# ChASE-library/ChASE

Measured on AMD Instinct MI355X. Metric: chebyshev_filter_hemm_gflops, higher is better.
Workload: dtype complex f64

## Files before the change

### chase_amd/capi.py

```python
import ctypes as C
import os
import numpy as np

_HERE = os.path.dirname(os.path.abspath(__file__))
LIB_PATH = os.environ.get("CHASE_HIP_LIB") or os.path.join(_HERE, "lib", "libchase_hip.so")


class ChaseHipError(RuntimeError):
    def __init__(self, code, where, text=""):
        super().__init__(f"{where} failed with status {code}: {text}")
        self.code = code


def _load():
    if not os.path.exists(LIB_PATH):
        raise ImportError(
            f"{LIB_PATH} not found: build it with `make` (or `python -c 'import __graft_entry__ as g; g.build()'`). "
            "chase_amd has no CPU fallback.")
    try:
        import torch
    except Exception:
        pass
    return C.CDLL(LIB_PATH, mode=C.RTLD_GLOBAL)

# ... 166 lines not shown
        return DeviceArray(self, host.shape, dt).upload(host)

    def timer_start(self):
        check(lib.chase_hip_timer_start(self.h), "timer_start")

    def timer_stop(self):
        ms = C.c_float()
        check(lib.chase_hip_timer_stop(self.h, C.byref(ms)), "timer_stop")
        return ms.value

    def gemm(self, opA, m, n, k, alpha, A, lda, B, ldb, beta, Cm, ldc, cplx):
        op = opA.encode()[0:1]
        if cplx:
            check(lib.chase_hip_gemm_z(self.h, op, m, n, k, _z2(alpha), A, lda, B, ldb, _z2(beta), Cm, ldc), "gemm_z")
        else:
            check(lib.chase_hip_gemm_d(self.h, op, m, n, k, float(alpha), A, lda, B, ldb, float(beta), Cm, ldc),
                  "gemm_d")

    def gemm32(self, opA, m, n, k, alpha, A, lda, B, ldb, beta, Cm, ldc, cplx, split=False):
        op = opA.encode()[0:1]
        if cplx:
            f = lib.chase_hip_gemm_c_bf16x3 if split else lib.chase_hip_gemm_c
            check(f(self.h, op, m, n, k, _c2(alpha), A, lda, B, ldb, _c2(beta), Cm, ldc), "gemm_c")
        else:
            f = lib.chase_hip_gemm_s_bf16x3 if split else lib.chase_hip_gemm_s
            check(f(self.h, op, m, n, k, float(alpha), A, lda, B, ldb, float(beta), Cm, ldc), "gemm_s")

    def gemm32w(self, opA, m, n, k, alpha, A, lda, B, ldb, beta, Cm, ldc, cplx, split=False):
        op = opA.encode()[0:1]
        if cplx:
            f = lib.chase_hip_gemm_cz_bf16x3 if split else lib.chase_hip_gemm_cz
            check(f(self.h, op, m, n, k, _z2(alpha), A, lda, B, ldb, _z2(beta), Cm, ldc), "gemm_cz")
        else:
            f = lib.chase_hip_gemm_sd_bf16x3 if split else lib.chase_hip_gemm_sd
            check(f(self.h, op, m, n, k, float(alpha), A, lda, B, ldb, float(beta), Cm, ldc), "gemm_sd")

    def bf16x3_pack_bytes(self, m, k, cplx):
        b = c_size_t()
        check(lib.chase_hip_bf16x3_pack_bytes(int(cplx), m, k, C.byref(b)), "bf16x3_pack_bytes")
        return b.value

    def bf16x3_pack(self, m, k, A, lda, packed, cplx, src_f64=False):
        check(lib.chase_hip_bf16x3_pack(self.h, int(cplx), int(src_f64), m, k, A, lda, packed), "bf16x3_pack")

    def bf16x3_pack_diag(self, n, H64, ldh, packed, cplx):
        check(lib.chase_hip_bf16x3_pack_diag(self.h, int(cplx), n, H64, ldh, packed), "bf16x3_pack_diag")

    def gemm32p(self, m, n, k, alpha, packedA, B, ldb, beta, Cm, ldc, cplx):
        if cplx:
            check(lib.chase_hip_gemm_c_bf16x3p(self.h, m, n, k, _c2(alpha), packedA, B, ldb, _c2(beta), Cm, ldc), "gemm_c_bf16x3p")
        else:
            check(lib.chase_hip_gemm_s_bf16x3p(self.h, m, n, k, float(alpha), packedA, B, ldb, float(beta), Cm, ldc),
                  "gemm_s_bf16x3p")

    def set_gemm_min_rounds(self, rounds):
        check(lib.chase_hip_ctx_set_gemm_min_rounds(self.h, int(rounds)), "ctx_set_gemm_min_rounds")

    def gemm_sp_counters(self, reset=False):
        w, s, p = C.c_ulonglong(), C.c_ulonglong(), C.c_ulonglong()
        check(lib.chase_hip_ctx_gemm_sp_counters(self.h, C.byref(w), C.byref(s), C.byref(p), int(reset)), "ctx_gemm_sp_counters")
        return w.value, s.value, p.value

    def diag_list_d2s(self, H, ldh, Hs, ldhs, rows, cols, cnt, cplx):
        check(lib.chase_hip_diag_list_d2s(self.h, int(cplx), H, ldh, Hs, ldhs, rows, cols, cnt), "diag_list_d2s")

    def convert_d2s(self, m, n, src, ld_src, dst, ld_dst, cplx):
        check(lib.chase_hip_convert_d2s(self.h, int(cplx), m, n, src, ld_src, dst, ld_dst), "convert_d2s")

    def convert_s2d(self, m, n, src, ld_src, dst, ld_dst, cplx):
        check(lib.chase_hip_convert_s2d(self.h, int(cplx), m, n, src, ld_src, dst, ld_dst), "convert_s2d")

    def diag_d2s(self, n, H, ldh, Hs, ldhs, cplx):
        check(lib.chase_hip_diag_d2s(self.h, int(cplx), n, H, ldh, Hs, ldhs), "diag_d2s")

    def to_single(self, dA):
        cplx = dA.dtype == np.complex128
        out = self.empty(dA.shape, np.complex64 if cplx else np.float32)
        self.convert_d2s(dA.shape[0], dA.shape[1], dA.ptr, dA.ld, out.ptr, out.ld, cplx)
        return out

    def to_double(self, dA):
        cplx = dA.dtype == np.complex64
        out = self.empty(dA.shape, np.complex128 if cplx else np.float64)
        self.convert_s2d(dA.shape[0], dA.shape[1], dA.ptr, dA.ld, out.ptr, out.ld, cplx)
        return out

    def hash64(self, ptr, m, n, ld, cplx):
        h = C.c_ulonglong()
        check(lib.chase_hip_hash64(self.h, int(cplx), m, n, ptr, ld, C.byref(h)), "hash64")
        return h.value

    def gen_clement(self, N, cplx, scale=1.0, perturb=0.0, seed=42):
        dH = self.empty((N, N), np.complex128 if cplx else np.float64)
        check(lib.chase_hip_gen_clement(self.h, int(cplx), dH.ptr, N, N, N, N, N, 1, 0, 0, N, 1, 0, 0, float(scale),
                                        float(perturb), seed), "gen_clement")
        return dH

    def load_matrix(self, path, N, cplx):
        dH = self.empty((N, N), np.complex128 if cplx else np.float64)
        check(lib.chase_hip_load_matrix_shard(self.h, str(path).encode(), int(cplx), N, N, N, N, 1, 0, N, 1, 0, dH.ptr, N),
              "load_matrix_shard")
        return dH

    def save_matrix(self, path, dA):
        cplx = dA.dtype == np.complex128
        check(lib.chase_hip_save_matrix(self.h, str(path).encode(), int(cplx), dA.shape[0],
# ... 154 lines not shown


def tape_get(solver):
    p, n = P(c_double)(), c_size_t()
    check(lib.chase_hip_solver_tape_data(solver.h, C.byref(p), C.byref(n)), "tape_data")
    return np.ctypeslib.as_array(p, shape=(n.value,)).copy() if n.value else np.zeros(0)


def tape_load(solver, tape):
    t = np.ascontiguousarray(tape, dtype=np.float64)
    check(lib.chase_hip_solver_tape_load(solver.h, t.ctypes.data, t.size), "tape_load")


def gemm_counters(ctx, phase, reset=False):
    a, b, n = c_double(), c_double(), C.c_ulonglong()
    check(lib.chase_hip_ctx_gemm_counters(ctx.h, phase, C.byref(a), C.byref(b), C.byref(n), int(reset)), "gemm_counters")
    return a.value, b.value, n.value


class GemmLaunch(C.Structure):
    _fields_ = [(f, c_int) for f in ("row0", "col0", "k0", "m", "n", "k", "beta_one", "bn_cols", "narrow", "m3", "ragged",
                                     "glds_ok", "gm", "gn")] + \
               [("full_tiles", c_long), ("tail_tiles", c_long)] + \
               [(f, c_int) for f in ("tail_sk", "tail_kchunk", "group_rows", "forced_split")] + \
               [("slab_bytes", c_size_t), ("plane_bytes", c_size_t)]

    def as_dict(self):
        return {k: getattr(self, k) for k, _ in self._fields_}


_sig("chase_hip_gemm_plan", c_int, c_int, c_char, c_int, c_int, c_int, c_long, c_long, c_int, c_int, c_int, c_int,
     P(GemmLaunch), c_int)


def gemm_plan(cplx, op, m, n, k, lda=None, ldb=None, aligned=True, phase=0, num_cu=256, min_rounds=0):
    lda = (m if op == "N" else k) if lda is None else lda
    ldb = k if ldb is None else ldb
    args = (int(cplx), op.encode(), m, n, k, max(lda, 1), max(ldb, 1), int(aligned), phase, num_cu, min_rounds)
    cnt = lib.chase_hip_gemm_plan(*args, None, 0)
    if cnt < 0:
        check(cnt, "gemm_plan")
    out = (GemmLaunch * max(cnt, 1))()
    assert lib.chase_hip_gemm_plan(*args, out, cnt) == cnt
    return [out[i].as_dict() for i in range(cnt)]


class GemmSpLaunch(C.Structure):
    _fields_ = [(n, c_int) for n in ("bn", "gm", "gn", "sk", "kchunk", "min_piece_k")] + [("slab_bytes", c_size_t)]

    def as_dict(self):
        return {k: getattr(self, k) for k, _ in self._fields_}


_sig("chase_hip_gemm_sp_plan", c_int, c_int, c_int, c_char, c_int, c_int, c_int, c_int, c_int, P(GemmSpLaunch))
_sig("chase_hip_gemm_sp_workspace_bytes", c_size_t, c_int, c_int, c_char, c_int, c_int, c_int, c_int, c_int)
_sig("chase_hip_ctx_gemm_sp_counters", c_int, c_void_p, P(C.c_ulonglong), P(C.c_ulonglong), P(C.c_ulonglong), c_int)


def gemm_sp_plan(cplx, op, m, n, k, split=False, num_cu=256, min_rounds=0):
    out = GemmSpLaunch()
    check(lib.chase_hip_gemm_sp_plan(int(split), int(cplx), op.encode(), m, n, k, num_cu, min_rounds, C.byref(out)), "gemm_sp_plan")
    return out.as_dict()


def gemm_sp_workspace_bytes(cplx, op, m, n, k, split=False, num_cu=256, min_rounds=0):
    return lib.chase_hip_gemm_sp_workspace_bytes(int(split), int(cplx), op.encode(), m, n, k, num_cu, min_rounds)


class Solver:

    def __init__(self, ctx, H, nev, nex, V=None, h_on_device_ptr=None, N=None, cplx=None):
        self.ctx = ctx
        if h_on_device_ptr is None:
            assert H.flags.f_contiguous and H.ndim == 2 and H.shape[0] == H.shape[1]
            self.cplx = bool(np.iscomplexobj(H))
            self.N = H.shape[0]
            self.H = H
            hptr, on_dev = H.ctypes.data, 0
        else:
            self.cplx, self.N, self.H = bool(cplx), int(N), None
            hptr, on_dev = h_on_device_ptr, 1
        self.nev, self.nex = nev, nex
        dt = np.complex128 if self.cplx else np.float64
        self.V = np.zeros((self.N, nev + nex), dtype=dt, order="F") if V is None else V
        assert self.V.flags.f_contiguous and self.V.dtype == dt
        self.ritzv = np.zeros(nev + nex, dtype=np.float64)
        h = c_void_p()
        check(lib.chase_hip_solver_create(C.byref(h), ctx.h, int(self.cplx), self.N, nev, nex, hptr, self.N,
                                          self.V.ctypes.data, self.N, self.ritzv.ctypes.data, on_dev),
              "solver_create")
        self.h = h

    def close(self):
        if self.h:
            lib.chase_hip_solver_destroy(self.h)
            self.h = None

    def set(self, **kw):
        for k, v in kw.items():
            check(lib.chase_hip_solver_set(self.h, k.encode(), float(v)), f"solver_set({k})")

    def get(self, key):
        v = c_double()
        check(lib.chase_hip_solver_get(self.h, key.encode(), C.byref(v)), f"solver_get({key})")
        return v.value

# ... 125 lines not shown
```

### chase_amd/csrc/capi_core.hip

```cpp
#include <hip/hip_runtime.h>
#include <cstdlib>
#include <cstdio>
#include <cstring>
#include <string>
#include "../../include/chase_hip.h"
#include "ctx.h"
#include "kernels.h"
#include "gemm_sp_frame.h"

namespace chase_hip {
thread_local std::string g_last_error;
int set_error(int code, const char* what)
{
    g_last_error = what ? what : "";
    return code;
}
int hip_fail(hipError_t e, const char* where)
{
    char buf[512];
    snprintf(buf, sizeof buf, "%s: %s", where, hipGetErrorString(e));
    g_last_error = buf;
    return -(int)e;
}
}
// ... 262 lines not shown
}

int chase_hip_gemm_c_bf16x3(chase_hip_ctx* c, char opA, int m, int n, int k, const float alpha[2], const void* A, long lda,
                            const void* B, long ldb, const float beta[2], void* C, long ldc)
{
    if (!c) return set_error(CHASE_HIP_EINVAL, "ctx == NULL");
    if (!alpha || !beta) return set_error(CHASE_HIP_EINVAL, "gemm_c: NULL alpha/beta");
    return gemm32(c, true, opA, m, n, k, alpha, (const float*)A, lda, (const float*)B, ldb, beta, (float*)C, ldc, true);
}

int chase_hip_bf16x3_pack_bytes(int cplx, int m, int k, size_t* bytes)
{
    if (!bytes) return set_error(CHASE_HIP_EINVAL, "bf16x3_pack_bytes: bytes == NULL");
    if (m < 0 || k < 0) return set_error(CHASE_HIP_EINVAL, "bf16x3_pack_bytes: negative dimension");
    *bytes = bf16x3_pack_bytes(cplx != 0, m, k);
    return 0;
}

int chase_hip_bf16x3_pack(chase_hip_ctx* c, int cplx, int src_f64, int m, int k, const void* A, long lda, void* packed)
{
    if (!c) return set_error(CHASE_HIP_EINVAL, "bf16x3_pack: NULL ctx");
    (void)hipSetDevice(c->device);
    if (c->oplog_on) c->oplog_add("bf16x3_pack", m, k, 0, 0);
    if (m < 0 || k < 0 || lda < m) return set_error(CHASE_HIP_EINVAL, "bf16x3_pack: bad shape");
    if (m == 0 || k == 0) return 0;
    if (!A || !packed) return set_error(CHASE_HIP_EINVAL, "bf16x3_pack: NULL matrix");
    if (((uintptr_t)packed & 15) != 0) return set_error(CHASE_HIP_EINVAL, "bf16x3_pack: packed must be 16-byte aligned");
    int e = bf16x3_pack(c->stream, cplx != 0, src_f64 != 0, m, k, A, lda, packed);
    if (e) return hip_fail((hipError_t)e, "bf16x3_pack launch");
    return 0;
}

int chase_hip_bf16x3_pack_diag(chase_hip_ctx* c, int cplx, int n, const void* H64, long ldh, void* packed)
{
    if (!c) return set_error(CHASE_HIP_EINVAL, "bf16x3_pack_diag: NULL ctx");
    (void)hipSetDevice(c->device);
    if (c->oplog_on) c->oplog_add("bf16x3_pack_diag", n, 0, 0, 0);
    if (n < 0 || ldh < n) return set_error(CHASE_HIP_EINVAL, "bf16x3_pack_diag: bad shape");
    if (n == 0) return 0;
    if (!H64 || !packed) return set_error(CHASE_HIP_EINVAL, "bf16x3_pack_diag: NULL argument");
    int e = bf16x3_pack_diag(c->stream, cplx != 0, n, (const double*)H64, ldh, packed);
    if (e) return hip_fail((hipError_t)e, "bf16x3_pack_diag launch");
    return 0;
}

static int gemm32p(chase_hip_ctx* c, bool cplx, int m, int n, int k, const float* alpha, const void* packedA, const float* B, long ldb,
                   const float* beta, float* C, long ldc)
{
    (void)hipSetDevice(c->device);
    int rc = check_gemm('N', m, n, k, packedA, m, B, ldb, C, ldc);
    if (rc || m == 0 || n == 0) return rc;
    if (k > 0 && ((uintptr_t)packedA & 15) != 0) return set_error(CHASE_HIP_EINVAL, "gemm_bf16x3p: packedA must be 16-byte aligned");
    if (c->oplog_on) c->oplog_add(cplx ? "gemm_c3pN" : "gemm_s3pN", m, n, k, c->phase * 100);
    int e = gemm_bf16x3p(c->stream, cplx, m, n, k, alpha, packedA, B, ldb, beta, C, ldc, c->num_cu, c->phase == 1 ? 1 : 0);
    if (e) return hip_fail((hipError_t)e, "gemm_bf16x3p launch");
    return 0;
}

int chase_hip_gemm_s_bf16x3p(chase_hip_ctx* c, int m, int n, int k, float alpha, const void* packedA, const float* B, long ldb,
                             float beta, float* C, long ldc)
{
    if (!c) return set_error(CHASE_HIP_EINVAL, "ctx == NULL");
    return gemm32p(c, false, m, n, k, &alpha, packedA, B, ldb, &beta, C, ldc);
}

int chase_hip_gemm_c_bf16x3p(chase_hip_ctx* c, int m, int n, int k, const float alpha[2], const void* packedA, const void* B, long ldb,
                             const float beta[2], void* C, long ldc)
{
    if (!c) return set_error(CHASE_HIP_EINVAL, "ctx == NULL");
    if (!alpha || !beta) return set_error(CHASE_HIP_EINVAL, "gemm_c_bf16x3p: NULL alpha/beta");
    return gemm32p(c, true, m, n, k, alpha, packedA, (const float*)B, ldb, beta, (float*)C, ldc);
}

static int gemm32w(chase_hip_ctx* c, bool cplx, char opA, int m, int n, int k, const double* alpha, const float* A, long lda,
                   const float* B, long ldb, const double* beta, double* C, long ldc, bool split = false)
{
    (void)hipSetDevice(c->device);
    const bool opn = opA == 'N' || opA == 'n';
    const bool opc = opA == 'C' || opA == 'c' || (!cplx && (opA == 'T' || opA == 't'));
    if (!opn && !opc)
        return set_error(CHASE_HIP_EINVAL, cplx ? "gemm_cz: opA must be 'N' or 'C'" : "gemm_sd: opA must be 'N', 'C' or 'T'");
    int rc = check_gemm(opA, m, n, k, A, lda, B, ldb, C, ldc);
    if (rc || m == 0 || n == 0) return rc;
    if (c->oplog_on) {
        const char* name = split ? (cplx ? (opn ? "gemm_cz3N" : "gemm_cz3C") : (opn ? "gemm_sd3N" : "gemm_sd3C"))
                                 : (cplx ? (opn ? "gemm_czN" : "gemm_czC") : (opn ? "gemm_sdN" : "gemm_sdC"));
        c->oplog_add(name, m, n, k, c->phase * 100);
    }
    if (c->gemm_min_rounds > 0) {
        const size_t need = chase_hip_gemm_sp_workspace_bytes(split, cplx, opA, m, n, k, c->num_cu, c->gemm_min_rounds);
        if (need && (rc = c->ensure_ws((need + ((size_t)32 << 20) - 1) & ~(((size_t)32 << 20) - 1)))) return rc;
    }
    int pieces = 1;
    int e = (split ? gemm_bf16x3w : gemm_f32w)(c->stream, cplx, opA, m, n, k, alpha, A, lda, B, ldb, beta, C, ldc, c->num_cu,
                                               c->phase == 1 ? 1 : 0, (double*)c->ws, c->ws_bytes, c->gemm_min_rounds, &pieces);
    if (e == GEMM_F32_EOP) return set_error(CHASE_HIP_EINVAL, "gemm_sd / gemm_cz: bad opA");
    if (e == GEMM_F64_EWORKSPACE)
        return set_error(CHASE_HIP_EINVAL, "gemm_sd / gemm_cz: split-K workspace smaller than gemm_sp_workspace_bytes for this shape");
    if (e) return hip_fail((hipError_t)e, split ? "gemm_bf16x3w launch" : "gemm_f32w launch");
    ++c->sp_wide_calls;
    if (pieces > 1) { ++c->sp_split_calls; c->sp_pieces += (unsigned long long)pieces; }
    return 0;
}

int chase_hip_gemm_sd(chase_hip_ctx* c, char opA, int m, int n, int k, double alpha, const float* A, long lda, const float* B,
                      long ldb, double beta, double* C, long ldc)
{
    if (!c) return set_error(CHASE_HIP_EINVAL, "ctx == NULL");
// ... 146 lines not shown
```

### chase_amd/csrc/ctx.h

```cpp
#pragma once
#include <hip/hip_runtime.h>
#include <stddef.h>
#include <string>
#include <vector>

struct chase_hip_ctx {
    int device = 0;
    int num_cu = 0;
    int clock_khz = 0;
    size_t hbm_bytes = 0;
    char name[128] = {0};
    hipStream_t stream = nullptr;
    bool own_stream = false;
    hipEvent_t ev0 = nullptr, ev1 = nullptr;
    int phase = 0;
    double flops_model[4] = {0, 0, 0, 0}, flops_exec[4] = {0, 0, 0, 0};
    unsigned long long gemm_calls[4] = {0, 0, 0, 0};
    int gemm_min_rounds = 0;
    unsigned long long sp_wide_calls = 0, sp_split_calls = 0, sp_pieces = 0;
    void* ws = nullptr;
    size_t ws_bytes = 0;
    enum { BUF_TINV = 0, BUF_PANEL, BUF_SCAL, BUF_LAMBDA, BUF_RR, BUF_EIG, BUF_STEDC, BUF_APPLYQ, NBUF };
    void* bufs[NBUF] = {};
    size_t buf_bytes[NBUF] = {};
    void* hstage = nullptr;
    size_t hstage_bytes = 0;

    bool oplog_on = false;
    int oplog_mute = 0;
    std::vector<std::string> oplog;
    std::string oplog_text;
    void oplog_add(const char* name, long a, long b, long c, long d);

    int ensure_ws(size_t bytes);
    int ensure_buf(int idx, size_t bytes);
    int ensure_hstage(size_t bytes);
    int gemm(bool cplx, char opA, int m, int n, int k, const double* alpha, const double* A, long lda, const double* B,
             long ldb, const double* beta, double* C, long ldc);
};

namespace chase_hip {
int set_error(int code, const char* what);
int hip_fail(hipError_t e, const char* where);
}
```

### chase_amd/csrc/gemm_mfma_bf16x3p.hip

```cpp
#include "gemm_sp_frame.h"

namespace chase_hip {
namespace {

using namespace sp_frame;

typedef __bf16 bf16x8 __attribute__((ext_vector_type(8)));
typedef unsigned u32x4 __attribute__((ext_vector_type(4)));

constexpr int BK = 16;
constexpr int PA = 2 * BM;

__host__ __device__ __forceinline__ int piece(int row, int h) { return 2 * row + (h ^ (((row >> 2) ^ (row >> 3)) & 1)); }

__device__ __forceinline__ void split1(float v, __bf16& a1, __bf16& a2, __bf16& a3)
{
    a1 = (__bf16)v;
    const float r1 = v - (float)a1;
    a2 = (__bf16)r1;
    const float r2 = r1 - (float)a2;
    a3 = (__bf16)r2;
}

__device__ __forceinline__ void split3(const float* x, int st, u32x4& p1, u32x4& p2, u32x4& p3)
{
    bf16x8 a1, a2, a3;
    #pragma unroll
    for (int e = 0; e < 8; ++e) {
        __bf16 s1, s2, s3;
        split1(x[st * e], s1, s2, s3);
        a1[e] = s1; a2[e] = s2; a3[e] = s3;
    }
    p1 = __builtin_bit_cast(u32x4, a1); p2 = __builtin_bit_cast(u32x4, a2); p3 = __builtin_bit_cast(u32x4, a3);
}


template <bool CPLX, class S>
__global__ __launch_bounds__(256) void bf16x3_pack_kernel(int m, int k, const S* __restrict__ A, long lda, u32x4* __restrict__ out)
{
    constexpr int E = CPLX ? 2 : 1;
    const int tid = threadIdx.x, r = tid % BM, h = tid / BM;
    const long t = blockIdx.x, T = gridDim.x, p = blockIdx.y;
    const long row = p * BM + r, kg = t * BK + 8 * h;
    float x[8 * E];
    #pragma unroll
    for (int e = 0; e < 8; ++e) {
        #pragma unroll
        for (int c = 0; c < E; ++c) x[E * e + c] = 0.f;
        if (row < m && kg + e < k) {
            const S* q = A + E * (row + (kg + e) * lda);
            #pragma unroll
            for (int c = 0; c < E; ++c) x[E * e + c] = (float)q[c];
        }
    }
    u32x4* d = out + (p * T + t) * (3 * E * PA) + piece(r, h);
    #pragma unroll
    for (int c = 0; c < E; ++c) {
        u32x4 p1, p2, p3;
        split3(x + c, E, p1, p2, p3);
        d[(3 * c) * PA] = p1; d[(3 * c + 1) * PA] = p2; d[(3 * c + 2) * PA] = p3;
    }
}

template <bool CPLX>
__global__ __launch_bounds__(256) void bf16x3_pack_diag_kernel(int n, const double* __restrict__ H, long ldh, unsigned short* __restrict__ out)
{
    constexpr int E = CPLX ? 2 : 1;
    const long i = (long)blockIdx.x * 256 + threadIdx.x;
    if (i >= n) return;
    const long T = ((long)n + BK - 1) / BK, p = i / BM, t = i / BK;
    const int r = (int)(i % BM), h = (int)(i % BK) / 8, e = (int)(i % 8);
    unsigned short* d = out + 8 * ((p * T + t) * (3 * E * PA) + piece(r, h)) + e;
    const double* q = H + E * (i + i * ldh);
    #pragma unroll
    for (int c = 0; c < E; ++c) {
        __bf16 s1, s2, s3;
        split1((float)q[c], s1, s2, s3);
        d[8L * (3 * c) * PA] = __builtin_bit_cast(unsigned short, s1);
        d[8L * (3 * c + 1) * PA] = __builtin_bit_cast(unsigned short, s2);
        d[8L * (3 * c + 2) * PA] = __builtin_bit_cast(unsigned short, s3);
    }
}


template <bool CPLX, int WN, int TAG, bool WIDE = false>
__global__ __launch_bounds__(256, 2) void gemm_bf16x3p_kernel(const Args a)
{
// ... 194 lines not shown
```

### chase_amd/csrc/kernels.h

```cpp
#pragma once
#include <hip/hip_runtime.h>
#include <stddef.h>

struct chase_hip_gemm_launch;

namespace chase_hip {

int gemm_f64(hipStream_t st, bool cplx, char opA, int m, int n, int k, const double* alpha, const double* A, long lda,
             const double* B, long ldb, const double* beta, double* C, long ldc, double* ws, size_t ws_bytes,
             int num_cu, int tag = 0, int device = 0, double* exec_flops = nullptr, int min_rounds = 0);
constexpr size_t GEMM_WS_CAP = (size_t)640 << 20;
size_t gemm_f64_ws_need(bool cplx, char opA, int m, int n, int k, int num_cu, int min_rounds = 0);
constexpr int GEMM_F64_EWORKSPACE = -77001;
int gemm3m_enabled();
void gemm3m_set(int on);
int gemm_f64_plan(bool cplx, char opA, int m, int n, int k, long lda, long ldb, bool aligned16, int tag, int num_cu, int min_rounds,
                  chase_hip_gemm_launch* out, int max_out);

constexpr int GEMM_F32_EOP = -77002;
int gemm_f32(hipStream_t st, bool cplx, char opA, int m, int n, int k, const float* alpha, const float* A, long lda, const float* B,
             long ldb, const float* beta, float* C, long ldc, int num_cu, int tag = 0);
int gemm_f32w(hipStream_t st, bool cplx, char opA, int m, int n, int k, const double* alpha, const float* A, long lda,
              const float* B, long ldb, const double* beta, double* C, long ldc, int num_cu, int tag = 0, double* ws = nullptr,
              size_t ws_bytes = 0, int min_rounds = 0, int* pieces = nullptr);
int gemm_bf16x3(hipStream_t st, bool cplx, char opA, int m, int n, int k, const float* alpha, const float* A, long lda, const float* B,
                long ldb, const float* beta, float* C, long ldc, int num_cu, int tag = 0);
int gemm_bf16x3w(hipStream_t st, bool cplx, char opA, int m, int n, int k, const double* alpha, const float* A, long lda,
                 const float* B, long ldb, const double* beta, double* C, long ldc, int num_cu, int tag = 0, double* ws = nullptr,
                 size_t ws_bytes = 0, int min_rounds = 0, int* pieces = nullptr);
size_t bf16x3_pack_bytes(bool cplx, int m, int k);
int bf16x3_pack(hipStream_t st, bool cplx, bool src_f64, int m, int k, const void* A, long lda, void* packed);
int bf16x3_pack_diag(hipStream_t st, bool cplx, int n, const double* H, long ldh, void* packed);
int gemm_bf16x3p(hipStream_t st, bool cplx, int m, int n, int k, const float* alpha, const void* packedA, const float* B, long ldb,
                 const float* beta, float* C, long ldc, int num_cu, int tag = 0);
int sp_slab_reduce(hipStream_t st, bool cplx, int m, int n, int sk, const double* S, long lds, long slab_stride, const double* alpha,
                   const double* beta, double* C, long ldc);

int mfma_f64_peak(hipStream_t st, double* out, int blocks, int iters);
int stream_copy(hipStream_t st, void* dst, const void* src, size_t bytes);

int shift_diag(hipStream_t st, double* H, long ld, int n, int ept, double shift);
int shift_list(hipStream_t st, double* H, long ld, const int* rows, const int* cols, int cnt, int ept, double shift);
int shift_diag_dev(hipStream_t st, double* A, long ld, int n, int ept, const double* nrmf_dev, double factor);
int abs_trace(hipStream_t st, const double* A, long ld, int n, int ept, double* out_dev);
int copy2d(hipStream_t st, const double* src, long ld_src_d, double* dst, long ld_dst_d, long md, int ncols);
int swap_cols(hipStream_t st, double* a, double* b, long md);
int rows_indexed(hipStream_t st, bool cplx, const double* in, long ld_in, double* out, long ld_out, const int* idx_dev,
                 int np, int ncols, int scatter);
int hash64(hipStream_t st, const double* x, long ld_d, long md, int ncols, unsigned long long* out_dev);
int tri_mask_bc(hipStream_t st, bool cplx, double* H, long ldh, int mloc, int nloc, long mb, int pr, int pi, long nb, int pc,
                int pj, int keep_upper);
int conj_transpose_add(hipStream_t st, bool cplx, const double* P, long ldp, int nr, int nc, const int* rowmap_dev,
                       const int* colmap_dev, double* H, long ldh);
int copy_cols_indexed(hipStream_t st, const double* src, long ld_src_d, double* dst, long ld_dst_d, long md,
                      const int* src_idx_dev, const int* dst_idx_dev, int cnt);
int copy_cols_indexed_range(hipStream_t st, const double* src, long ld_src_d, double* dst, long ld_dst_d, long md,
                            const int* src_idx_dev, int dst0, int cnt);
int resid_norms(hipStream_t st, const double* W, long ldw_d, const double* V, long ldv_d, const double* lambda_dev,
                long md, int ncols, double* out_dev, int do_sqrt);
int sqrt_inplace(hipStream_t st, double* x, int n);
int col_dot(hipStream_t st, bool cplx, const double* X, long ldx_d, const double* Y, long ldy_d, int m, int ncols,
            double* out_dev);
int col_axpy(hipStream_t st, bool cplx, const double* a_dev, int a_is_real, int a_stride, double sgn, const double* X,
             long ldx_d, double* Y, long ldy_d, int m, int ncols);
int col_scal(hipStream_t st, const double* a_dev, int inv, double* X, long ldx_d, long md, int ncols);
int scale_rows(hipStream_t st, double* X, long ldx_d, long row0_d, long md, int ncols, double s);
int scale_rows_bc(hipStream_t st, double* X, long ldx_d, long m, int ncols, int ept, long g0, long nb, int p, int q, double s);
int conj_inplace(hipStream_t st, double* X, long ldx_d, int m, int ncols);
int pack_upper(hipStream_t st, const double* A, long lda, int n, int ept, double* P);
int unpack_upper(hipStream_t st, double* P, int n, int ept, double* A, long lda);
int mirror_upper(hipStream_t st, double* A, long lda, int n, int ept);
int mirror_lower(hipStream_t st, double* A, long lda, int n, int ept, int zero_diag_imag = 1);
int convert_d2s(hipStream_t st, const double* src, long ld_src, float* dst, long ld_dst, long ms, int ncols);
int convert_s2d(hipStream_t st, const float* src, long ld_src, double* dst, long ld_dst, long ms, int ncols);
int diag_d2s(hipStream_t st, const double* H, long ldh, float* Hs, long ldhs, int n, int ept);
int diag_list_d2s(hipStream_t st, const double* H, long ldh, float* Hs, long ldhs, const int* rows, const int* cols, int cnt, int ept);

int fill_normal(hipStream_t st, bool cplx, double* X, long ldx, int m, int n, long grow0, long gcol0, long gld,
                unsigned long long seed, int mb = 0, int pr = 1, int pi = 0);
int gen_clement(hipStream_t st, bool cplx, double* H, long ldh, int mloc, int nloc, long N, int mb, int pr, int pi,
                long roff, int nb, int pc, int pj, long coff, double scale, double perturb, unsigned long long seed);
int gen_bse(hipStream_t st, bool cplx, double* H, long ldh, int mloc, int nloc, long N, int mb, int pr, int pi, int nb,
            int pc, int pj, double dmin, double dmax, double offdiag, unsigned long long seed);

}
struct chase_hip_ctx;
namespace chase_hip {
// ... 7 lines not shown
```

### include/chase_hip.h

```cpp
#ifndef CHASE_HIP_H
#define CHASE_HIP_H

#include <stddef.h>

#ifdef __cplusplus
extern "C" {
#endif

#define CHASE_HIP_OK 0
#define CHASE_HIP_EINVAL (-1001)
#define CHASE_HIP_ENODEV (-1002)
#define CHASE_HIP_ENOMEM (-1003)
#define CHASE_HIP_ENOTCONV (-1004)
#define CHASE_HIP_ECOMM (-1005)
#define CHASE_HIP_ELAPACK (-1006)
#define CHASE_HIP_EIO (-1007)

typedef struct chase_hip_ctx chase_hip_ctx;

int chase_hip_ctx_create(chase_hip_ctx** out, int device, void* stream);
int chase_hip_ctx_destroy(chase_hip_ctx* ctx);
int chase_hip_ctx_sync(chase_hip_ctx* ctx);
void* chase_hip_ctx_stream(chase_hip_ctx* ctx);
int chase_hip_ctx_oplog(chase_hip_ctx* ctx, int on);
int chase_hip_ctx_oplog_mute(chase_hip_ctx* ctx, int delta);
const char* chase_hip_ctx_oplog_text(chase_hip_ctx* ctx);
const char* chase_hip_last_error(void);
int chase_hip_device_info(chase_hip_ctx* ctx, int* num_cu, int* clock_khz, size_t* hbm_bytes, char* name,
                          int name_len);
int chase_hip_device_bus_id(chase_hip_ctx* ctx, char* out, int len);
const char* chase_hip_version(void);
int chase_hip_device_count(void);

int chase_hip_malloc(chase_hip_ctx* ctx, void** dev, size_t bytes);
int chase_hip_free(chase_hip_ctx* ctx, void* dev);
int chase_hip_memcpy_h2d(chase_hip_ctx* ctx, void* dev, const void* host, size_t bytes);
int chase_hip_memcpy_d2h(chase_hip_ctx* ctx, void* host, const void* dev, size_t bytes);
int chase_hip_memcpy_d2d(chase_hip_ctx* ctx, void* dst, const void* src, size_t bytes);
int chase_hip_memset(chase_hip_ctx* ctx, void* dev, int value, size_t bytes);
int chase_hip_timer_start(chase_hip_ctx* ctx);
int chase_hip_timer_stop(chase_hip_ctx* ctx, float* ms);

int chase_hip_gemm_d(chase_hip_ctx* ctx, char opA, int m, int n, int k, double alpha, const double* A, long lda,
                     const double* B, long ldb, double beta, double* C, long ldc);
int chase_hip_gemm_z(chase_hip_ctx* ctx, char opA, int m, int n, int k, const double alpha[2], const void* A,
                     long lda, const void* B, long ldb, const double beta[2], void* C, long ldc);
int chase_hip_gemm_s(chase_hip_ctx* ctx, char opA, int m, int n, int k, float alpha, const float* A, long lda, const float* B,
                     long ldb, float beta, float* C, long ldc);
int chase_hip_gemm_c(chase_hip_ctx* ctx, char opA, int m, int n, int k, const float alpha[2], const void* A, long lda,
                     const void* B, long ldb, const float beta[2], void* C, long ldc);
int chase_hip_gemm_sd(chase_hip_ctx* ctx, char opA, int m, int n, int k, double alpha, const float* A, long lda, const float* B,
                      long ldb, double beta, double* C, long ldc);
int chase_hip_gemm_cz(chase_hip_ctx* ctx, char opA, int m, int n, int k, const double alpha[2], const void* A, long lda,
                      const void* B, long ldb, const double beta[2], void* C, long ldc);
int chase_hip_gemm_s_bf16x3(chase_hip_ctx* ctx, char opA, int m, int n, int k, float alpha, const float* A, long lda,
                            const float* B, long ldb, float beta, float* C, long ldc);
int chase_hip_gemm_c_bf16x3(chase_hip_ctx* ctx, char opA, int m, int n, int k, const float alpha[2], const void* A, long lda,
                            const void* B, long ldb, const float beta[2], void* C, long ldc);
int chase_hip_gemm_sd_bf16x3(chase_hip_ctx* ctx, char opA, int m, int n, int k, double alpha, const float* A, long lda,
                             const float* B, long ldb, double beta, double* C, long ldc);
int chase_hip_gemm_cz_bf16x3(chase_hip_ctx* ctx, char opA, int m, int n, int k, const double alpha[2], const void* A, long lda,
                             const void* B, long ldb, const double beta[2], void* C, long ldc);

int chase_hip_bf16x3_pack_bytes(int cplx, int m, int k, size_t* bytes);
int chase_hip_bf16x3_pack(chase_hip_ctx* ctx, int cplx, int src_f64, int m, int k, const void* A, long lda, void* packed);
int chase_hip_bf16x3_pack_diag(chase_hip_ctx* ctx, int cplx, int n, const void* H64, long ldh, void* packed);
int chase_hip_gemm_s_bf16x3p(chase_hip_ctx* ctx, int m, int n, int k, float alpha, const void* packedA, const float* B, long ldb,
                             float beta, float* C, long ldc);
int chase_hip_gemm_c_bf16x3p(chase_hip_ctx* ctx, int m, int n, int k, const float alpha[2], const void* packedA, const void* B,
                             long ldb, const float beta[2], void* C, long ldc);

typedef struct chase_hip_gemm_sp_launch {
    int bn;
    int gm, gn;
    int sk, kchunk;
    int min_piece_k;
    size_t slab_bytes;
} chase_hip_gemm_sp_launch;
int chase_hip_gemm_sp_plan(int bf16x3, int cplx, char opA, int m, int n, int k, int num_cu, int min_rounds,
                           chase_hip_gemm_sp_launch* out);
size_t chase_hip_gemm_sp_workspace_bytes(int bf16x3, int cplx, char opA, int m, int n, int k, int num_cu, int min_rounds);
int chase_hip_ctx_gemm_sp_counters(chase_hip_ctx* ctx, unsigned long long* wide_calls, unsigned long long* split_calls,
                                   unsigned long long* pieces, int reset);

size_t chase_hip_gemm_workspace_bytes(int cplx, char opA, int m, int n, int k, int num_cu, int min_rounds);
typedef struct chase_hip_gemm_launch {
    int row0, col0, k0;
    int m, n, k;
    int beta_one;
    int bn_cols;
    int narrow;
    int m3;
    int ragged;
    int glds_ok;
    int gm, gn;
    long full_tiles;
    long tail_tiles;
    int tail_sk, tail_kchunk;
    int group_rows;
    int forced_split;
    size_t slab_bytes;
    size_t plane_bytes;
} chase_hip_gemm_launch;
int chase_hip_gemm_plan(int cplx, char opA, int m, int n, int k, long lda, long ldb, int aligned16, int phase, int num_cu,
                        int min_rounds, chase_hip_gemm_launch* out, int max_out);
int chase_hip_gemm3m_enabled(void);
int chase_hip_set_gemm3m(int on);
int chase_hip_ctx_gemm_counters(chase_hip_ctx* ctx, int phase, double* flops_model, double* flops_executed,
                                unsigned long long* calls, int reset);
int chase_hip_mfma_f64_peak(chase_hip_ctx* ctx, double* tflops);
int chase_hip_hbm_copy_peak(chase_hip_ctx* ctx, size_t bytes, double* gbps);

int chase_hip_ctx_set_phase(chase_hip_ctx* ctx, int phase);
int chase_hip_ctx_set_gemm_min_rounds(chase_hip_ctx* ctx, int rounds);

int chase_hip_fill_normal(chase_hip_ctx* ctx, int cplx, int m, int n, void* X, long ldx, long grow0, long gcol0,
                          long gld, unsigned long long seed);
int chase_hip_fill_normal_bc(chase_hip_ctx* ctx, int cplx, int m, int n, void* X, long ldx, long gld, int mb, int pr,
                             int pi, unsigned long long seed);
int chase_hip_rows_indexed(chase_hip_ctx* ctx, int cplx, const void* in, long ld_in, void* out, long ld_out,
                           const int* idx_dev, int np, int ncols, int scatter);
int chase_hip_hash64(chase_hip_ctx* ctx, int cplx, int m, int n, const void* A, long lda, unsigned long long* out_host);
int chase_hip_cols_indexed(chase_hip_ctx* ctx, int cplx, int m, const void* in, long ld_in, void* out, long ld_out,
// ... 83 lines not shown
```

Before: 100,700.

## Pre-split B into bf16x3 image and stream tiles via direct global-to-LDS loads

Packed bf16x3 GEMMs now first run a pack kernel that splits the fp32 B operand into three bf16 planes, stored in a tile-ordered image held in a new context buffer. A new MFMA kernel then streams both packed A and packed B into LDS with global_load_lds_dwordx4 through a three-stage pipeline, interleaving the copies with MFMA work. This is meant to remove the per-tile B splitting and the register staging from the main loop. In exchange it adds a separate pack pass, extra memory traffic and workspace for the B image, and inline assembly that depends on the hardware.

Measured after the change: 100,600. Within noise of the previous version (-0.1%).

```diff
diff --git a/chase_amd/capi.py b/chase_amd/capi.py
--- a/chase_amd/capi.py
+++ b/chase_amd/capi.py
@@ -242,6 +242,9 @@
         else:
             check(lib.chase_hip_gemm_s_bf16x3p(self.h, m, n, k, float(alpha), packedA, B, ldb, float(beta), Cm, ldc),
                   "gemm_s_bf16x3p")
+
+    def bf16x3_pack_b(self, n, k, B, ldb, bn, image, cplx):
+        check(lib.chase_hip_bf16x3_pack_b(self.h, int(cplx), n, k, B, ldb, bn, image), "bf16x3_pack_b")
 
     def set_gemm_min_rounds(self, rounds):
         check(lib.chase_hip_ctx_set_gemm_min_rounds(self.h, int(rounds)), "ctx_set_gemm_min_rounds")
@@ -502,6 +505,27 @@
         return {k: getattr(self, k) for k, _ in self._fields_}
 
 
+class Bf16x3DmaLaunch(C.Structure):
+    _fields_ = [(n, c_int) for n in ("bn", "threads", "stages", "planes", "gm", "gn", "steps", "b_ranges")] + \
+               [(n, c_size_t) for n in ("lds_bytes", "a_bytes", "b_bytes", "a_step_bytes", "b_step_bytes", "a_off")] + \
+               [("b_off", c_size_t * 2)]
+
+    def as_dict(self):
+        d = {k: getattr(self, k) for k, _ in self._fields_}
+        d["b_off"] = list(self.b_off)[:self.b_ranges]
+        return d
+
+
+_sig("chase_hip_bf16x3_dma_plan", c_int, c_int, c_int, c_int, c_int, c_int, c_int, c_int, c_int, P(Bf16x3DmaLaunch))
+_sig("chase_hip_bf16x3_pack_b", c_int, c_void_p, c_int, c_int, c_int, c_void_p, c_long, c_int, c_void_p)
+
+
+def bf16x3_dma_plan(cplx, m, n, k, num_cu=256, tile=(0, 0), step=0):
+    out = Bf16x3DmaLaunch()
+    check(lib.chase_hip_bf16x3_dma_plan(int(cplx), m, n, k, num_cu, tile[0], tile[1], step, C.byref(out)), "bf16x3_dma_plan")
+    return out.as_dict()
+
+
 _sig("chase_hip_gemm_sp_plan", c_int, c_int, c_int, c_char, c_int, c_int, c_int, c_int, c_int, P(GemmSpLaunch))
 _sig("chase_hip_gemm_sp_workspace_bytes", c_size_t, c_int, c_int, c_char, c_int, c_int, c_int, c_int, c_int)
 _sig("chase_hip_ctx_gemm_sp_counters", c_int, c_void_p, P(C.c_ulonglong), P(C.c_ulonglong), P(C.c_ulonglong), c_int)
diff --git a/chase_amd/csrc/capi_core.hip b/chase_amd/csrc/capi_core.hip
--- a/chase_amd/csrc/capi_core.hip
+++ b/chase_amd/csrc/capi_core.hip
@@ -338,8 +338,38 @@
     if (rc || m == 0 || n == 0) return rc;
     if (k > 0 && ((uintptr_t)packedA & 15) != 0) return set_error(CHASE_HIP_EINVAL, "gemm_bf16x3p: packedA must be 16-byte aligned");
     if (c->oplog_on) c->oplog_add(cplx ? "gemm_c3pN" : "gemm_s3pN", m, n, k, c->phase * 100);
-    int e = gemm_bf16x3p(c->stream, cplx, m, n, k, alpha, packedA, B, ldb, beta, C, ldc, c->num_cu, c->phase == 1 ? 1 : 0);
-    if (e) return hip_fail((hipError_t)e, "gemm_bf16x3p launch");
+    const size_t need = bf16x3_dma_plan(cplx, m, n, k, c->num_cu).b_bytes;
+    if (need && (rc = c->ensure_buf(chase_hip_ctx::BUF_SPB, (need + ((size_t)32 << 20) - 1) & ~(((size_t)32 << 20) - 1)))) return rc;
+    int e = gemm_bf16x3d(c->stream, cplx, m, n, k, alpha, packedA, B, ldb, beta, C, ldc, c->num_cu, c->phase == 1 ? 1 : 0,
+                         c->bufs[chase_hip_ctx::BUF_SPB], c->buf_bytes[chase_hip_ctx::BUF_SPB]);
+    if (e) return hip_fail((hipError_t)e, "gemm_bf16x3d launch");
+    return 0;
+}
+
+int chase_hip_bf16x3_dma_plan(int cplx, int m, int n, int k, int num_cu, int tm, int tn, int t, chase_hip_bf16x3_dma_launch* out)
+{
+    if (m < 0 || n < 0 || k < 0 || !out) return set_error(CHASE_HIP_EINVAL, "bf16x3_dma_plan: bad argument");
+    const Bf16x3DmaPlan p = bf16x3_dma_plan(cplx != 0, m, n, k, num_cu);
+    if (tm < 0 || tn < 0 || t < 0 || (p.gm && tm >= p.gm) || (p.gn && tn >= p.gn) || (p.steps && t >= p.steps))
+        return set_error(CHASE_HIP_EINVAL, "bf16x3_dma_plan: no such tile or K step");
+    out->bn = p.bn; out->threads = p.threads; out->stages = p.stages; out->planes = p.planes;
+    out->gm = p.gm; out->gn = p.gn; out->steps = p.steps; out->b_ranges = p.b_ranges;
+    out->lds_bytes = p.lds_bytes; out->a_bytes = p.a_bytes; out->b_bytes = p.b_bytes;
+    out->a_step_bytes = p.a_step_bytes; out->b_step_bytes = p.b_step_bytes;
+    bf16x3_dma_read(p, tm, tn, t, &out->a_off, out->b_off);
+    return 0;
+}
+
+int chase_hip_bf16x3_pack_b(chase_hip_ctx* c, int cplx, int n, int k, const void* B, long ldb, int bn, void* image)
+{
+    if (!c) return set_error(CHASE_HIP_EINVAL, "bf16x3_pack_b: NULL ctx");
+    (void)hipSetDevice(c->device);
+    if (n < 0 || k < 0 || ldb < k || (bn != 64 && bn != 128)) return set_error(CHASE_HIP_EINVAL, "bf16x3_pack_b: bad shape");
+    if (n == 0 || k == 0) return 0;
+    if (!B || !image) return set_error(CHASE_HIP_EINVAL, "bf16x3_pack_b: NULL matrix");
+    if (((uintptr_t)image & 15) != 0) return set_error(CHASE_HIP_EINVAL, "bf16x3_pack_b: image must be 16-byte aligned");
+    int e = bf16x3_pack_b(c->stream, cplx != 0, n, k, (const float*)B, ldb, bn, image);
+    if (e) return hip_fail((hipError_t)e, "bf16x3_pack_b launch");
     return 0;
 }
 
diff --git a/chase_amd/csrc/ctx.h b/chase_amd/csrc/ctx.h
--- a/chase_amd/csrc/ctx.h
+++ b/chase_amd/csrc/ctx.h
@@ -20,7 +20,7 @@
     unsigned long long sp_wide_calls = 0, sp_split_calls = 0, sp_pieces = 0;
     void* ws = nullptr;
     size_t ws_bytes = 0;
-    enum { BUF_TINV = 0, BUF_PANEL, BUF_SCAL, BUF_LAMBDA, BUF_RR, BUF_EIG, BUF_STEDC, BUF_APPLYQ, NBUF };
+    enum { BUF_TINV = 0, BUF_PANEL, BUF_SCAL, BUF_LAMBDA, BUF_RR, BUF_EIG, BUF_STEDC, BUF_APPLYQ, BUF_SPB, NBUF };
     void* bufs[NBUF] = {};
     size_t buf_bytes[NBUF] = {};
     void* hstage = nullptr;
diff --git a/chase_amd/csrc/gemm_bf16x3_split.h b/chase_amd/csrc/gemm_bf16x3_split.h
--- /dev/null
+++ b/chase_amd/csrc/gemm_bf16x3_split.h
@@ -0,0 +1,41 @@
+#pragma once
+#include <hip/hip_runtime.h>
+
+namespace chase_hip {
+namespace bf16x3_split {
+
+typedef __bf16 bf16x8 __attribute__((ext_vector_type(8)));
+typedef unsigned u32x4 __attribute__((ext_vector_type(4)));
+
+constexpr int BK = 16;
+
+__host__ __device__ __forceinline__ int piece(int row, int h) { return 2 * row + (h ^ (((row >> 2) ^ (row >> 3)) & 1)); }
+
+constexpr int A_PIECES = 256, B_PIECES = 128, B_COLS = 64;
+__host__ __device__ __forceinline__ long a_block(long p, long T, long t, int planes) { return (p * T + t) * planes * A_PIECES; }
+__host__ __device__ __forceinline__ long b_block(long c, long T, long t, int planes) { return (c * T + t) * planes * B_PIECES; }
+__host__ __device__ __forceinline__ long b_blocks(long n, int bn) { return (n + bn - 1) / bn * (bn / B_COLS); }
+
+__device__ __forceinline__ void split1(float v, __bf16& a1, __bf16& a2, __bf16& a3)
+{
+    a1 = (__bf16)v;
+    const float r1 = v - (float)a1;
+    a2 = (__bf16)r1;
+    const float r2 = r1 - (float)a2;
+    a3 = (__bf16)r2;
+}
+
+__device__ __forceinline__ void split3(const float* x, int st, u32x4& p1, u32x4& p2, u32x4& p3)
+{
+    bf16x8 a1, a2, a3;
+    #pragma unroll
+    for (int e = 0; e < 8; ++e) {
+        __bf16 s1, s2, s3;
+        split1(x[st * e], s1, s2, s3);
+        a1[e] = s1; a2[e] = s2; a3[e] = s3;
+    }
+    p1 = __builtin_bit_cast(u32x4, a1); p2 = __builtin_bit_cast(u32x4, a2); p3 = __builtin_bit_cast(u32x4, a3);
+}
+
+}
+}
diff --git a/chase_amd/csrc/gemm_mfma_bf16x3d.hip b/chase_amd/csrc/gemm_mfma_bf16x3d.hip
--- /dev/null
+++ b/chase_amd/csrc/gemm_mfma_bf16x3d.hip
@@ -0,0 +1,292 @@
+#include "gemm_sp_frame.h"
+#include "gemm_bf16x3_split.h"
+#include <atomic>
+
+namespace chase_hip {
+namespace {
+
+using namespace sp_frame;
+using namespace bf16x3_split;
+
+constexpr int STAGES = 3;
+constexpr int MAX_DEVICES = 64;
+
+__device__ __forceinline__ void glds_copy(unsigned voff, const char* sbase, const u32x4* lds_dst)
+{
+    const unsigned dst = (unsigned)(size_t)(__attribute__((address_space(3))) const void*)lds_dst;
+    asm volatile("s_mov_b32 m0, %2\n\ts_nop 0\n\tglobal_load_lds_dwordx4 %0, %1" :: "v"(voff), "s"(sbase), "s"(dst) : "memory");
+}
+
+
+template <bool CPLX>
+__global__ __launch_bounds__(256) void bf16x3_pack_b_kernel(int n, int k, const float* __restrict__ B, long ldb, int vec,
+                                                            u32x4* __restrict__ out)
+{
+    constexpr int E = CPLX ? 2 : 1;
+    const int tid = threadIdx.x, oct = tid & 7, cl = tid >> 3;
+    const long T = ((long)k + BK - 1) / BK, t = 4L * blockIdx.x + (oct >> 1), c = blockIdx.y;
+    const int h = oct & 1;
+    if (t >= T) return;
+    const long kg = t * BK + 8 * h;
+    #pragma unroll
+    for (int pass = 0; pass < 2; ++pass) {
+        const int jb = cl + 32 * pass;
+        const long col = c * B_COLS + jb;
+        float x[8 * E];
+        #pragma unroll
+        for (int q = 0; q < 8 * E; ++q) x[q] = 0.f;
+        if (col < n) {
+            const float* p = B + E * (kg + col * ldb);
+            if (vec && kg + 8 <= k) {
+                #pragma unroll
+                for (int q = 0; q < 2 * E; ++q) {
+                    const float4 v = ((const float4*)p)[q];
+                    x[4 * q] = v.x; x[4 * q + 1] = v.y; x[4 * q + 2] = v.z; x[4 * q + 3] = v.w;
+                }
+            } else {
+                #pragma unroll
+                for (int e = 0; e < 8; ++e)
+                    if (kg + e < k) {
+                        #pragma unroll
+                        for (int s = 0; s < E; ++s) x[E * e + s] = p[E * e + s];
+                    }
+            }
+        }
+        u32x4* d = out + b_block(c, T, t, 3 * E) + piece(jb, h);
+        #pragma unroll
+        for (int s = 0; s < E; ++s) {
+            u32x4 p1, p2, p3;
+            split3(x + s, E, p1, p2, p3);
+            d[(3 * s) * B_PIECES] = p1; d[(3 * s + 1) * B_PIECES] = p2; d[(3 * s + 2) * B_PIECES] = p3;
+        }
+    }
+}
+
+
+__host__ __device__ constexpr int stage_pieces(bool cplx, int bn) { return (cplx ? 6 : 3) * (A_PIECES + (bn / B_COLS) * B_PIECES); }
+
+template <bool CPLX, int WN, int NW, int TAG, bool WIDE = false>
+__global__ __launch_bounds__(64 * NW, 2) void gemm_bf16x3d_kernel(const Args a)
+{
+    static_assert(!WIDE, "narrow form only: fp32 C and scalars");
+    constexpr int BN = 32 * WN * (NW / 2);
+    constexpr int E = CPLX ? 2 : 1;
+    constexpr int NH = BN / B_COLS;
+    static_assert(BN == 64 || BN == 128, "tile columns");
+    constexpr int STAGE = stage_pieces(CPLX, BN);
+    constexpr int UA = 3 * E * A_PIECES / 64, UB = 3 * E * B_PIECES / 64;
+    constexpr int U = UA + NH * UB;
+    constexpr int G = (U + NW - 1) / NW;
+    constexpr int GMIN = U / NW;
+    extern __shared__ __attribute__((aligned(16))) u32x4 lds[];
+
+    const Place at = place<BN>(a);
+    const int wm = at.wm, wn = at.wn, lr = at.lr, lh = at.lh;
+    const int wv = __builtin_amdgcn_readfirstlane(at.tid >> 6);
+    const int T = (a.k + BK - 1) / BK;
+
+    f32x16 acc[2][WN][E];
+    #pragma unroll
+    for (int i = 0; i < 2; ++i)
+        #pragma unroll
+        for (int j = 0; j < WN; ++j)
+            #pragma unroll
+            for (int p = 0; p < E; ++p)
+                #pragma unroll
+                for (int r = 0; r < 16; ++r) acc[i][j][p][r] = 0.f;
+
+    const char* src[G];
+    const unsigned voff = (unsigned)(at.tid & 63) * 16u;
+    #pragma unroll
+    for (int i = 0; i < G; ++i) {
+        const int u = wv + NW * i;
+        if (u < UA) {
+            src[i] = (const char*)a.A + (a_block(at.m0 / BM, T, 0, 3 * E) + 64L * u) * 16;
+        } else {
+            const int ub = u - UA, hh = ub / UB, r = ub - hh * UB;
+            src[i] = (const char*)a.B + (b_block(at.n0 / B_COLS + hh, T, 0, 3 * E) + 64L * r) * 16;
+        }
+    }
+    auto issue_one = [&](int i, int st) __attribute__((always_inline)) {
+        const int u = wv + NW * i;
+        if (G == GMIN || i < GMIN || u < U) {
+            glds_copy(voff, src[i], lds + st * STAGE + 64 * u);
+            src[i] += (u < UA ? 3 * E * A_PIECES : 3 * E * B_PIECES) * 16;
+        }
+    };
+
+    auto mfma = [](const u32x4& x, const u32x4& y, f32x16& c) {
+        c = __builtin_amdgcn_mfma_f32_32x32x16_bf16(__builtin_bit_cast(bf16x8, x), __builtin_bit_cast(bf16x8, y), c, 0, 0, 0);
+    };
+    auto prod6 = [&](const u32x4* x, const u32x4* y, f32x16& c) {
+        mfma(x[2], y[0], c); mfma(x[1], y[1], c); mfma(x[0], y[2], c);
+        mfma(x[1], y[0], c); mfma(x[0], y[1], c); mfma(x[0], y[0], c);
+    };
+    constexpr int NG = CPLX ? 8 : 2 * WN;
+    const int cw = wn * (32 * WN);
+    const int offA = piece(wm * 64 + lr, lh);
+    const int offB = 3 * E * A_PIECES + (cw / B_COLS) * (3 * E * B_PIECES) + piece(cw % B_COLS + lr, lh);
+    auto step = [&](int st, int sf, auto fill_c) __attribute__((always_inline)) {
+        constexpr bool FILL = decltype(fill_c)::value;
+        const u32x4* As = lds + st * STAGE + offA;
+        const u32x4* Bs = lds + st * STAGE + offB;
+        auto hook = [&](int g) __attribute__((always_inline)) {
+            if constexpr (FILL) {
+                __builtin_amdgcn_sched_barrier(0);
+                #pragma unroll
+                for (int i = g * G / NG; i < (g + 1) * G / NG; ++i) issue_one(i, sf);
+                __builtin_amdgcn_sched_barrier(0);
+            }
+        };
+        if constexpr (CPLX) {
+            static_assert(WN == 1, "complex waves are 64 x 32");
+            u32x4 fb[2][3];
+            #pragma unroll
+            for (int p = 0; p < 2; ++p)
+                #pragma unroll
+                for (int s = 0; s < 3; ++s) fb[p][s] = Bs[(3 * p + s) * B_PIECES];
+            #pragma unroll
+            for (int i = 0; i < 2; ++i) {
+                u32x4 fa[2][3];
+                #pragma unroll
+                for (int p = 0; p < 2; ++p)
+                    #pragma unroll
+                    for (int s = 0; s < 3; ++s) fa[p][s] = As[(3 * p + s) * A_PIECES + 64 * i];
+                hook(4 * i);
+                prod6(fa[0], fb[0], acc[i][0][0]);
+                hook(4 * i + 1);
+                prod6(fa[0], fb[1], acc[i][0][1]);
+                hook(4 * i + 2);
+                prod6(fa[1], fb[0], acc[i][0][1]);
+                #pragma unroll
+                for (int s = 0; s < 3; ++s) fa[1][s] ^= 0x80008000u;
+                hook(4 * i + 3);
+                prod6(fa[1], fb[1], acc[i][0][0]);
+            }
+        } else {
+            u32x4 fb[WN][3];
+            #pragma unroll
+            for (int j = 0; j < WN; ++j)
+                #pragma unroll
+                for (int s = 0; s < 3; ++s) fb[j][s] = Bs[s * B_PIECES + 64 * j];
+            #pragma unroll
+            for (int i = 0; i < 2; ++i) {
+                u32x4 fa[3];
+                #pragma unroll
+                for (int s = 0; s < 3; ++s) fa[s] = As[s * A_PIECES + 64 * i];
+                #pragma unroll
+                for (int j = 0; j < WN; ++j) {
+                    hook(i * WN + j);
+                    prod6(fa, fb[j], acc[i][j][0]);
+                }
+            }
+        }
+    };
+    auto publish = [&](bool ahead) __attribute__((always_inline)) {
+        if (ahead) asm volatile("s_waitcnt vmcnt(%0) lgkmcnt(0)" ::"n"(GMIN) : "memory");
+        else       asm volatile("s_waitcnt vmcnt(0) lgkmcnt(0)" ::: "memory");
+        __builtin_amdgcn_s_barrier();
+        asm volatile("" ::: "memory");
+    };
+
+    constexpr std::true_type yes{};
+    constexpr std::false_type no{};
+    #pragma unroll
+    for (int t = 0; t < 2; ++t)
+        if (t < T) {
+            #pragma unroll
+            for (int i = 0; i < G; ++i) issue_one(i, t);
+        }
+    int st = 0, t = 0;
+    for (; t + 2 < T; ++t) {
+        publish(true);
+        step(st, st == 0 ? 2 : st - 1, yes);
+        st = st == 2 ? 0 : st + 1;
+    }
+    for (; t < T; ++t) {
+        publish(t + 1 < T);
+        step(st, 0, no);
+        st = st == 2 ? 0 : st + 1;
+    }
+#include "gemm_sp_epilogue.h"
+}
+
+template <bool CPLX, int WN, int NW, int TAG>
+int launch_tag(hipStream_t st, const Args& a, int dev)
+{
+    constexpr int BN = 32 * WN * (NW / 2);
+    constexpr size_t lds_bytes = (size_t)STAGES * stage_pieces(CPLX, BN) * 16;
+    static std::atomic<bool> attr_set[MAX_DEVICES];
+    if (!attr_set[dev].load(std::memory_order_relaxed)) {
+        (void)hipFuncSetAttribute((const void*)gemm_bf16x3d_kernel<CPLX, WN, NW, TAG>, hipFuncAttributeMaxDynamicSharedMemorySize,
+                                  (int)lds_bytes);
+        attr_set[dev].store(true, std::memory_order_relaxed);
+    }
+    hipLaunchKernelGGL((gemm_bf16x3d_kernel<CPLX, WN, NW, TAG>), dim3(a.total), dim3(64 * NW), lds_bytes, st, a);
+    return (int)hipGetLastError();
+}
+
+template <bool CPLX, int WN, int NW>
+int launch(hipStream_t st, const Args& a, int tag)
+{
+    int dev = 0;
+    (void)hipGetDevice(&dev);
+    if (dev < 0 || dev >= MAX_DEVICES) dev = 0;
+    return tag == 1 ? launch_tag<CPLX, WN, NW, 1>(st, a, dev) : launch_tag<CPLX, WN, NW, 0>(st, a, dev);
+}
+
+}
+
+Bf16x3DmaPlan bf16x3_dma_plan(bool cplx, int m, int n, int k, int num_cu)
+{
+    Bf16x3DmaPlan p{};
+    p.bn = cplx ? (n <= 64 ? 64 : 128) : tile_cols(m, n, num_cu);
+    p.threads = (cplx && p.bn == 128) ? 512 : 256;
+    p.stages = STAGES;
+    p.planes = cplx ? 6 : 3;
+    p.gm = m > 0 ? (int)(((long)m + BM - 1) / BM) : 0;
+    p.gn = n > 0 ? (int)(((long)n + p.bn - 1) / p.bn) : 0;
+    p.steps = k > 0 ? (int)(((long)k + BK - 1) / BK) : 0;
+    p.lds_bytes = (size_t)STAGES * stage_pieces(cplx, p.bn) * 16;
+    p.a_bytes = bf16x3_pack_bytes(cplx, m, k);
+    p.b_bytes = (n > 0 && k > 0) ? (size_t)b_blocks(n, p.bn) * p.steps * p.planes * B_PIECES * 16 : 0;
+    p.a_step_bytes = (size_t)p.planes * A_PIECES * 16;
+    p.b_step_bytes = (size_t)p.planes * B_PIECES * 16;
+    p.b_ranges = p.bn / B_COLS;
+    return p;
+}
+
+void bf16x3_dma_read(const Bf16x3DmaPlan& p, int tm, int tn, int t, size_t* a_off, size_t b_off[2])
+{
+    *a_off = (size_t)a_block(tm, p.steps, t, p.planes) * 16;
+    for (int hh = 0; hh < 2; ++hh)
+        b_off[hh] = hh < p.b_ranges ? (size_t)b_block((long)tn * p.b_ranges + hh, p.steps, t, p.planes) * 16 : 0;
+}
+
+int bf16x3_pack_b(hipStream_t st, bool cplx, int n, int k, const float* B, long ldb, int bn, void* image)
+{
+    if (n <= 0 || k <= 0) return 0;
+    if (bn != 64 && bn != 128) return (int)hipErrorInvalidValue;
+    const long T = ((long)k + BK - 1) / BK, cb = b_blocks(n, bn);
+    if (cb > 65535) return (int)hipErrorInvalidValue;
+    const int vec = (al16(B) && (ldb & (cplx ? 1 : 3)) == 0) ? 1 : 0;
+    const dim3 grid((unsigned)((T + 3) / 4), (unsigned)cb);
+    if (cplx) hipLaunchKernelGGL(bf16x3_pack_b_kernel<true>, grid, dim3(256), 0, st, n, k, B, ldb, vec, (u32x4*)image);
+    else hipLaunchKernelGGL(bf16x3_pack_b_kernel<false>, grid, dim3(256), 0, st, n, k, B, ldb, vec, (u32x4*)image);
+    return (int)hipGetLastError();
+}
+
+int gemm_bf16x3d(hipStream_t st, bool cplx, int m, int n, int k, const float* alpha, const void* packedA, const float* B, long ldb,
+                 const float* beta, float* C, long ldc, int num_cu, int tag, void* image, size_t image_bytes)
+{
+    if (m <= 0 || n <= 0) return 0;
+    const Bf16x3DmaPlan p = bf16x3_dma_plan(cplx, m, n, k, num_cu);
+    if (p.b_bytes > image_bytes || (p.b_bytes && !image)) return GEMM_F64_EWORKSPACE;
+    if (const int e = bf16x3_pack_b(st, cplx, n, k, B, ldb, p.bn, image)) return e;
+    return narrow(cplx, 'N', m, n, k, alpha, (const float*)packedA, 0, (const float*)image, 0, beta, C, ldc, p.bn, [&](const Args& a) {
+        if (cplx) return p.bn == 64 ? launch<true, 1, 4>(st, a, tag) : launch<true, 1, 8>(st, a, tag);
+        return p.bn == 64 ? launch<false, 1, 4>(st, a, tag) : launch<false, 2, 4>(st, a, tag);
+    });
+}
+
+}
diff --git a/chase_amd/csrc/gemm_mfma_bf16x3p.hip b/chase_amd/csrc/gemm_mfma_bf16x3p.hip
--- a/chase_amd/csrc/gemm_mfma_bf16x3p.hip
+++ b/chase_amd/csrc/gemm_mfma_bf16x3p.hip
@@ -1,38 +1,13 @@
 #include "gemm_sp_frame.h"
+#include "gemm_bf16x3_split.h"
 
 namespace chase_hip {
 namespace {
 
 using namespace sp_frame;
-
-typedef __bf16 bf16x8 __attribute__((ext_vector_type(8)));
-typedef unsigned u32x4 __attribute__((ext_vector_type(4)));
-
-constexpr int BK = 16;
+using namespace bf16x3_split;
+
 constexpr int PA = 2 * BM;
-
-__host__ __device__ __forceinline__ int piece(int row, int h) { return 2 * row + (h ^ (((row >> 2) ^ (row >> 3)) & 1)); }
-
-__device__ __forceinline__ void split1(float v, __bf16& a1, __bf16& a2, __bf16& a3)
-{
-    a1 = (__bf16)v;
-    const float r1 = v - (float)a1;
-    a2 = (__bf16)r1;
-    const float r2 = r1 - (float)a2;
-    a3 = (__bf16)r2;
-}
-
-__device__ __forceinline__ void split3(const float* x, int st, u32x4& p1, u32x4& p2, u32x4& p3)
-{
-    bf16x8 a1, a2, a3;
-    #pragma unroll
-    for (int e = 0; e < 8; ++e) {
-        __bf16 s1, s2, s3;
-        split1(x[st * e], s1, s2, s3);
-        a1[e] = s1; a2[e] = s2; a3[e] = s3;
-    }
-    p1 = __builtin_bit_cast(u32x4, a1); p2 = __builtin_bit_cast(u32x4, a2); p3 = __builtin_bit_cast(u32x4, a3);
-}
 
 
 template <bool CPLX, class S>
diff --git a/chase_amd/csrc/kernels.h b/chase_amd/csrc/kernels.h
--- a/chase_amd/csrc/kernels.h
+++ b/chase_amd/csrc/kernels.h
@@ -33,6 +33,17 @@
 int bf16x3_pack_diag(hipStream_t st, bool cplx, int n, const double* H, long ldh, void* packed);
 int gemm_bf16x3p(hipStream_t st, bool cplx, int m, int n, int k, const float* alpha, const void* packedA, const float* B, long ldb,
                  const float* beta, float* C, long ldc, int num_cu, int tag = 0);
+struct Bf16x3DmaPlan {
+    int bn, threads, stages, planes;
+    int gm, gn, steps;
+    int b_ranges;
+    size_t lds_bytes, a_bytes, b_bytes, a_step_bytes, b_step_bytes;
+};
+Bf16x3DmaPlan bf16x3_dma_plan(bool cplx, int m, int n, int k, int num_cu);
+void bf16x3_dma_read(const Bf16x3DmaPlan& p, int tm, int tn, int t, size_t* a_off, size_t b_off[2]);
+int bf16x3_pack_b(hipStream_t st, bool cplx, int n, int k, const float* B, long ldb, int bn, void* image);
+int gemm_bf16x3d(hipStream_t st, bool cplx, int m, int n, int k, const float* alpha, const void* packedA, const float* B, long ldb,
+                 const float* beta, float* C, long ldc, int num_cu, int tag, void* image, size_t image_bytes);
 int sp_slab_reduce(hipStream_t st, bool cplx, int m, int n, int sk, const double* S, long lds, long slab_stride, const double* alpha,
                    const double* beta, double* C, long ldc);
 
diff --git a/include/chase_hip.h b/include/chase_hip.h
--- a/include/chase_hip.h
+++ b/include/chase_hip.h
@@ -69,6 +69,15 @@
                              float beta, float* C, long ldc);
 int chase_hip_gemm_c_bf16x3p(chase_hip_ctx* ctx, int m, int n, int k, const float alpha[2], const void* packedA, const void* B,
                              long ldb, const float beta[2], void* C, long ldc);
+
+typedef struct chase_hip_bf16x3_dma_launch {
+    int bn, threads, stages, planes;
+    int gm, gn, steps, b_ranges;
+    size_t lds_bytes, a_bytes, b_bytes, a_step_bytes, b_step_bytes;
+    size_t a_off, b_off[2];
+} chase_hip_bf16x3_dma_launch;
+int chase_hip_bf16x3_dma_plan(int cplx, int m, int n, int k, int num_cu, int tm, int tn, int t, chase_hip_bf16x3_dma_launch* out);
+int chase_hip_bf16x3_pack_b(chase_hip_ctx* ctx, int cplx, int n, int k, const void* B, long ldb, int bn, void* image);
 
 typedef struct chase_hip_gemm_sp_launch {
     int bn;
```
